# pnnl/nmrfit

Measured on AMD Instinct MI355X. Metric: objective evals/sec (swarm x grid x peaks), higher is better.
Workload: dtype f64

## Files before the change

### nmrfit_amd/csrc/ctx.hip

```cpp
#include "host_call.h"
#include "nmrfit_amd_diag.h"

#include <algorithm>
#include <cmath>
#include <cstdlib>
#include <new>

namespace nmrfit {

int ensure(nmrfit_ctx *ctx, double **buf, int64_t *cap, int64_t need)
{
    if (need <= *cap) return NMRFIT_OK;
    NMRFIT_HIP(hipStreamSynchronize(ctx->stream));
    if (*buf) NMRFIT_HIP(hipFree(*buf));
    *buf = nullptr;
    *cap = 0;
    int64_t n = need + need / 4 + 64;
    NMRFIT_HIP(hipMalloc((void **)buf, (size_t)n * sizeof(double)));
    *cap = n;
    return NMRFIT_OK;
}

void analyse_grid(const double *w, int64_t N, double *w0_out, double *wspan_out, double *lane_step_out, double *grid_dev_out)
{
    const double w0 = w[N / 2];
    double wspan = 0.0, lane_step = 0.0, grid_dev = 0.0;
    for (int64_t j = 0; j < N; ++j) wspan = std::fmax(wspan, std::fabs(w[j] - w0));
    if (N >= 2 * kChunk) {
        const double first = w[0] - w0, step = ((w[N - 1] - w0) - first) / (double)(N - 1);
        double dev = 0.0;
        for (int64_t j = 0; j < N; ++j) dev = std::fmax(dev, std::fabs((w[j] - w0) - (first + (double)j * step)));
        if (step != 0.0 && dev <= 1.0e-6 * std::fabs(step)) {
            lane_step = step * kWave;
            grid_dev = 2.0 * dev;
        }
    }
    *w0_out = w0;
    *wspan_out = wspan;
    *lane_step_out = lane_step;
    *grid_dev_out = grid_dev;
}

static bool variant_known(int variant)
{
    return variant == NMRFIT_VARIANT_DEFAULT || variant == NMRFIT_VARIANT_BASELINE || variant == NMRFIT_VARIANT_NOSKIP ||
           variant == NMRFIT_VARIANT_FARFIELD || variant == NMRFIT_VARIANT_NOREC || variant == NMRFIT_VARIANT_FARFIELD32;
}
static bool variant_built(int variant)
{
#ifdef NMRFIT_AB_BUILD
    return variant_known(variant);
#else
    return variant == NMRFIT_VARIANT_DEFAULT || variant == NMRFIT_VARIANT_FARFIELD || variant == NMRFIT_VARIANT_NOREC ||
           variant == NMRFIT_VARIANT_FARFIELD32;
#endif
}

}

using namespace nmrfit;

#pragma GCC visibility push(default)
extern "C" {

int nmrfit_ctx_create(int device, int64_t N, const double *w, const double *u, const double *v,
                      const double *weights, nmrfit_ctx **out)
{
    if (!out) {
        set_error("null out pointer");
        return NMRFIT_E_INVALID;
    }
    *out = nullptr;
    if (N <= 0 || !w || !u || !v || !weights) {
        set_error("nmrfit_ctx_create: N must be > 0 and w, u, v, weights non-null");
        return NMRFIT_E_INVALID;
    }
    DeviceInfo prop;
    int rc = use_device(device, &prop);
    if (rc != NMRFIT_OK) return rc;
    nmrfit_ctx *ctx = new (std::nothrow) nmrfit_ctx();
    if (!ctx) {
        set_error("out of host memory");
        return NMRFIT_E_INVALID;
    }
    ctx->device = device;
    ctx->compute_units = prop.cus;
    ctx->N = N;
    ctx->n_chunks = block_plan(N).n_chunks;
    if (const char *tw = getenv("NMRFIT_TARGET_WAVES")) ctx->target_waves = atoll(tw);
    if (getenv("NMRFIT_NO_WIDE_WORKGROUPS")) ctx->wide_workgroups = false;
    if (const char *dv = getenv("NMRFIT_DEFAULT_VARIANT")) {
        const int vnum = atoi(dv);
        if (variant_built(vnum)) ctx->variant = vnum;
    }
    analyse_grid(w, N, &ctx->w0, &ctx->wspan, &ctx->lane_step, &ctx->grid_dev);
    const size_t bytes = (size_t)N * sizeof(double);
    const size_t padded = (size_t)ctx->n_chunks * kChunk * sizeof(double);
    NMRFIT_HIP_OR(take_stream(device, &ctx->own_stream), nmrfit_ctx_destroy(ctx));
    ctx->stream = ctx->own_stream;
    NMRFIT_HIP_OR(hipEventCreate(&ctx->ev0), nmrfit_ctx_destroy(ctx));
    NMRFIT_HIP_OR(hipEventCreate(&ctx->ev1), nmrfit_ctx_destroy(ctx));
    Carver c;
    const size_t o_wc = c.take(padded), o_u = c.take(padded), o_v = c.take(padded), o_wt = c.take(padded);
    const size_t o_chunk = c.take((size_t)ctx->n_chunks * sizeof(double2)), o_stage = c.take(bytes);
    NMRFIT_HIP_OR(hipMalloc((void **)&ctx->d_block, c.total), nmrfit_ctx_destroy(ctx));
    NMRFIT_HIP_OR(hipMemsetAsync(ctx->d_block, 0, o_chunk, ctx->stream), nmrfit_ctx_destroy(ctx));
    unsigned char *base = reinterpret_cast<unsigned char *>(ctx->d_block);
    ctx->d_wc = reinterpret_cast<double *>(base + o_wc);
    ctx->d_u = reinterpret_cast<double *>(base + o_u);
    ctx->d_v = reinterpret_cast<double *>(base + o_v);
    ctx->d_wt = reinterpret_cast<double *>(base + o_wt);
    ctx->d_chunk = reinterpret_cast<double2 *>(base + o_chunk);
    ctx->d_stage = reinterpret_cast<double *>(base + o_stage);
    NMRFIT_HIP_OR(hipMemcpyAsync(ctx->d_stage, w, bytes, hipMemcpyHostToDevice, ctx->stream), nmrfit_ctx_destroy(ctx));
    rc = prepare_grid(ctx, ctx->d_stage);
    const double *host_arrays[] = {u, v, weights};
    double *dev_arrays[] = {ctx->d_u, ctx->d_v, ctx->d_wt};
    for (int a = 0; a < 3 && rc == NMRFIT_OK; ++a) {
        NMRFIT_HIP_OR(hipMemcpyAsync(ctx->d_stage, host_arrays[a], bytes, hipMemcpyHostToDevice, ctx->stream),
                      nmrfit_ctx_destroy(ctx));
        rc = scatter_grid(ctx, ctx->d_stage, dev_arrays[a]);
    }
    if (rc != NMRFIT_OK) {
        nmrfit_ctx_destroy(ctx);
        return rc;
    }
    NMRFIT_HIP_OR(hipStreamSynchronize(ctx->stream), nmrfit_ctx_destroy(ctx));
    *out = ctx;
    return NMRFIT_OK;
}

int nmrfit_ctx_destroy(nmrfit_ctx *ctx)
{
    if (!ctx) return NMRFIT_OK;
    (void)hipSetDevice(ctx->device);
    if (ctx->own_stream) {
        (void)hipStreamSynchronize(ctx->stream);
        if (ctx->stream != ctx->own_stream) (void)hipStreamSynchronize(ctx->own_stream);
    }
    void *bufs[] = {ctx->d_block , ctx->d_X, ctx->d_f, ctx->d_partial, ctx->d_R, ctx->d_lsq};
    for (void *b : bufs)
        if (b) (void)hipFree(b);
    if (ctx->ev0) (void)hipEventDestroy(ctx->ev0);
    if (ctx->ev1) (void)hipEventDestroy(ctx->ev1);
    (void)nmrfit_prof_enable(ctx, 0);
    if (ctx->own_stream) give_stream(ctx->device, ctx->own_stream);
    delete ctx;
    return NMRFIT_OK;
}

int nmrfit_ctx_set_weights(nmrfit_ctx *ctx, const double *weights)
{
    int rc = bind(ctx);
    if (rc != NMRFIT_OK) return rc;
    if (!weights) {
        set_error("null weights");
        return NMRFIT_E_INVALID;
    }
    NMRFIT_HIP(hipMemcpyAsync(ctx->d_stage, weights, (size_t)ctx->N * sizeof(double), hipMemcpyHostToDevice, ctx->stream));
    rc = scatter_grid(ctx, ctx->d_stage, ctx->d_wt);
    if (rc != NMRFIT_OK) return rc;
    NMRFIT_HIP(hipStreamSynchronize(ctx->stream));
    return NMRFIT_OK;
}

int nmrfit_ctx_synchronize(nmrfit_ctx *ctx)
{
    int rc = bind(ctx);
    if (rc != NMRFIT_OK) return rc;
    NMRFIT_HIP(hipStreamSynchronize(ctx->stream));
    return NMRFIT_OK;
}

int nmrfit_ctx_set_stream(nmrfit_ctx *ctx, void *hip_stream)
{
    int rc = bind(ctx);
    if (rc != NMRFIT_OK) return rc;
    NMRFIT_HIP(hipStreamSynchronize(ctx->stream));
    ctx->stream = hip_stream ? (hipStream_t)hip_stream : ctx->own_stream;
    return NMRFIT_OK;
}

int nmrfit_ctx_set_variant(nmrfit_ctx *ctx, int variant)
{
    if (!ctx || !variant_known(variant)) {
        set_error("bad context or variant");
        return NMRFIT_E_INVALID;
    }
    if (!variant_built(variant))
        return refuse(NMRFIT_E_UNSUPPORTED,
                      "this kernel variant is an A/B form: it exists in libnmrfit_amd_ab.so (nmrfit_amd/csrc/build.sh --ab) only");
    ctx->variant = variant;
    return NMRFIT_OK;
}

int nmrfit_ctx_n(const nmrfit_ctx *ctx, int64_t *N)
{
    if (!ctx || !N) {
        set_error("null argument");
        return NMRFIT_E_INVALID;
    }
    *N = ctx->N;
    return NMRFIT_OK;
}

int nmrfit_ctx_set_fit_im(nmrfit_ctx *ctx, int fit_im)
{
    const int rc = check_fit_im(ctx ? fit_im : -1);
    if (rc != NMRFIT_OK) return rc;
    ctx->fit_im = fit_im;
    return NMRFIT_OK;
}

int nmrfit_dev_alloc(nmrfit_ctx *ctx, int64_t bytes, void **dptr)
{
    int rc = bind(ctx);
    if (rc != NMRFIT_OK) return rc;
    if (!dptr || bytes < 0) {
        set_error("bad arguments to nmrfit_dev_alloc");
        return NMRFIT_E_INVALID;
    }
    *dptr = nullptr;
    if (bytes == 0) return NMRFIT_OK;
    NMRFIT_HIP(hipMalloc(dptr, (size_t)bytes));
    return NMRFIT_OK;
}

int nmrfit_dev_free(nmrfit_ctx *ctx, void *dptr)
{
    int rc = bind(ctx);
    if (rc != NMRFIT_OK) return rc;
    if (!dptr) return NMRFIT_OK;
    NMRFIT_HIP(hipStreamSynchronize(ctx->stream));
    NMRFIT_HIP(hipFree(dptr));
    return NMRFIT_OK;
}

static int ctx_memcpy(nmrfit_ctx *ctx, const char *who, void *dst, const void *src, int64_t bytes, hipMemcpyKind kind)
{
    int rc = bind(ctx);
    if (rc != NMRFIT_OK) return rc;
    if (bytes < 0 || (bytes > 0 && (!dst || !src))) return refuse(NMRFIT_E_INVALID, std::string("bad arguments to ") + who);
    if (bytes == 0) return NMRFIT_OK;
// ... 169 lines not shown
```

### nmrfit_amd/csrc/nmrfit_internal.h

```cpp
#pragma once
#include <hip/hip_runtime.h>
#include <stdint.h>
#include <string>
#include <vector>

#include "nmrfit_amd.h"

namespace nmrfit {

constexpr int kWave = 64;
constexpr int kWavesPerBlock = 4;
constexpr int kBlock = kWave * kWavesPerBlock;
#ifndef NMRFIT_POINTS
#define NMRFIT_POINTS 8
#endif
constexpr int kPointsPerLane = NMRFIT_POINTS;
constexpr int kChunk = kWave * kPointsPerLane;
constexpr int kMaxBlocks = 16;
struct BlockPlan {
    int64_t n_chunks;
    int blk_chunks;
    int64_t n_blocks;
    int64_t blk_len;
};
inline BlockPlan block_plan(int64_t N)
{
    BlockPlan p;
    p.n_chunks = (N + kChunk - 1) / kChunk;
    p.blk_chunks = (int)((p.n_chunks + kMaxBlocks - 1) / kMaxBlocks);
    p.n_blocks = (p.n_chunks + p.blk_chunks - 1) / p.blk_chunks;
    p.blk_len = (int64_t)p.blk_chunks * kChunk;
    return p;
}
constexpr int kMaxPeaks = 960;

__host__ __device__ inline int64_t grid_slot(int64_t j)
{
    const int64_t o = j & (int64_t)(kChunk - 1);
    const int64_t l = o & (int64_t)(kWave - 1), q = o >> 6;
    return (j - o) + (q >> 1) * (2 * kWave) + 2 * l + (q & 1);
}
static_assert(kWave == 64 && kPointsPerLane % 2 == 0, "grid_slot assumes wave64 and an even number of points per lane");

__device__ inline void chunk_minmax_wave(const double *wc, int64_t N, int64_t c, int lane, double2 *out)
{
    double lo = INFINITY, hi = -INFINITY;
    for (int q = 0; q < kPointsPerLane; ++q) {
        const int64_t j = c * kChunk + q * kWave + lane;
        if (j < N) {
            const double x = wc[grid_slot(j)];
            lo = fmin(lo, x);
            hi = fmax(hi, x);
        }
    }
    for (int off = 32; off > 0; off >>= 1) {
        lo = fmin(lo, __shfl_down(lo, off, kWave));
        hi = fmax(hi, __shfl_down(hi, off, kWave));
    }
    if (lane == 0) out[c] = make_double2(lo, hi);
}

struct PeakLor {
    double ihw;
    double c;
    double al;
    double ag2;
};
struct PeakFast {
    double ihs;
    double cs;
    double ia;
    double pad;
};
struct PeakWin {
    float lo;
    float hi;
};

void set_error(const std::string &msg);
void analyse_grid(const double *w, int64_t N, double *w0, double *wspan, double *lane_step, double *grid_dev);
struct DeviceInfo {
    bool known = false;
    int cus = 0;
    char arch[64] = {0};
};
int device_info_cached(int device, DeviceInfo *out);
int use_device(int device, DeviceInfo *info = nullptr);
int check_spectra_count(const char *who, int32_t S);
hipError_t take_stream(int device, hipStream_t *out);
void give_stream(int device, hipStream_t s);
int hip_fail(hipError_t e, const char *what, const char *file, int line);
int staged_d2h(int device, hipStream_t st, void *dst_host, const void *src_dev, size_t bytes);

#define NMRFIT_HIP(call)                                                        \
    do {                                                                        \
        hipError_t _e = (call);                                                 \
        if (_e != hipSuccess) return ::nmrfit::hip_fail(_e, #call, __FILE__, __LINE__); \
    } while (0)

struct LaunchGeom {
    int64_t waves = 0;
    int32_t nseg = 1;
    int64_t seg_len = 0;
    int32_t waves_per_workgroup = 4;
};

}

struct nmrfit_ctx {
    int device = -1;
    int compute_units = 0;
    hipStream_t stream = nullptr;
    hipStream_t own_stream = nullptr;
    int64_t N = 0;
    double w0 = 0.0;
    double wspan = 0.0;
    double lane_step = 0.0;
    double grid_dev = 0.0;
    int64_t target_waves = 0;
    bool wide_workgroups = true;
    void *d_block = nullptr;
    double *d_wc = nullptr;
    double *d_u = nullptr, *d_v = nullptr, *d_wt = nullptr;
    double2 *d_chunk = nullptr;
    double *d_stage = nullptr;
    int64_t n_chunks = 0;
    double *d_X = nullptr;
    int64_t cap_X = 0;
    double *d_f = nullptr;
    int64_t cap_f = 0;
    double *d_partial = nullptr;
    int64_t cap_partial = 0;
    double *d_R = nullptr;
    int64_t cap_R = 0;
    double *d_lsq = nullptr;
    int64_t cap_lsq = 0;
    hipEvent_t ev0 = nullptr, ev1 = nullptr;
    int variant = NMRFIT_VARIANT_DEFAULT;
    int fit_im = 0;
    nmrfit::LaunchGeom last;
    int64_t prof_cap = 0;
    std::vector<hipEvent_t> prof_k0, prof_k1, prof_marks;
    int64_t prof_nk = 0, prof_nm = 0;
    unsigned long long *d_clk = nullptr;
};

namespace nmrfit {
struct ObjectiveDeferred {
    bool needed = false;
    const double *partial = nullptr;
    int64_t n_blocks = 0;
    int fit_im = 0;
    bool pbest_done = false;
    bool tail_done = false;
    bool need_flush = false;
};
struct PsoFused;
constexpr int64_t kFusedMaxD = 400;
int launch_objective(nmrfit_ctx *ctx, int64_t S, int32_t P, const double *dX, double *df, double *dR,
                     ObjectiveDeferred *defer = nullptr, const PsoFused *fused = nullptr, int rows_fit_im = 0);
int ensure(nmrfit_ctx *ctx, double **buf, int64_t *cap, int64_t need);
int prepare_grid(nmrfit_ctx *ctx, const double *d_w_raw);
int scatter_grid(nmrfit_ctx *ctx, const double *d_src, double *d_dst);
int comm_all_gather(nmrfit_comm *c, hipStream_t stream, const double *d_send, int64_t n, const double **d_all);
nmrfit_ctx *comm_ctx(const nmrfit_comm *c);
bool comm_attach(nmrfit_comm *c);
void comm_detach(nmrfit_comm *c);
}
```

### nmrfit_amd/csrc/objective.hip

```cpp
#include "objective_launch.h"
#include "objective_lds.h"
#include "objective_math.h"

#include <algorithm>
#include <cmath>
#include <cstdio>
#include <cstdlib>

namespace nmrfit {
namespace {

__global__ void finalize_kernel(const double *__restrict__ partial, int64_t S, int64_t n_chunks, int64_t N,
                                int fit_im, double *__restrict__ f)
{
    const int64_t i = (int64_t)blockIdx.x * blockDim.x + threadIdx.x;
    if (i >= S) return;
    f[i] = finalize_value(partial + i * n_chunks * (fit_im ? 2 : 1), n_chunks, N, fit_im);
}

__global__ void finalize_rows_im_kernel(const double *__restrict__ partial, int64_t S, int64_t n_blocks, int64_t N,
                                        double *__restrict__ f2)
{
    const int64_t i = (int64_t)blockIdx.x * blockDim.x + threadIdx.x;
    if (i >= S) return;
// ... 45 lines not shown
{
    const int64_t N = ctx->N;
    hipLaunchKernelGGL(scatter_grid_kernel, dim3((unsigned)((N + 255) / 256)), dim3(256), 0, ctx->stream, d_src, N, d_dst);
    NMRFIT_HIP(hipGetLastError());
    return NMRFIT_OK;
}

constexpr size_t kStaticLds = kObjectiveStaticLds;
static_assert(kObjectiveStaticLds == (size_t)kWsumsCount * sizeof(double) + 64, "objective_launch.h and objective_math.h disagree");
namespace {
struct ResolvedLds {
    int variant;
    size_t lds;
    unsigned aux_off;
};
constexpr ResolvedLds resolve_lds(int variant, int32_t P, bool residual, int fit_im, int wpb, int slices, int rows)
{
    const bool want32 = variant == NMRFIT_VARIANT_FARFIELD32;
    if (want32) variant = NMRFIT_VARIANT_FARFIELD;
    const int np = P > 1 ? P : 1;
    const size_t room = 160 * 1024 - kStaticLds -
                        (rows ? (size_t)rows * (size_t)(4 + 3 * (int64_t)P) * sizeof(double) + 16 : 0);
    if (variant == NMRFIT_VARIANT_FARFIELD && objective_lds_layout(variant, residual, fit_im, np, wpb, slices).end + 16 > room)
        variant = NMRFIT_VARIANT_DEFAULT;
    if (variant == NMRFIT_VARIANT_DEFAULT && objective_lds_layout(variant, residual, fit_im, np, wpb, slices).end + 16 > room)
        variant = NMRFIT_VARIANT_NOREC;
    const ObjectiveLds at = objective_lds_layout(variant, residual, fit_im, np, wpb, slices);
    if (want32 && variant == NMRFIT_VARIANT_FARFIELD && !residual && fit_im == 0) variant = NMRFIT_VARIANT_FARFIELD32;
    return ResolvedLds{variant, at.end, fit_im != 0 ? (unsigned)at.tab : 0u};
}
struct LdsPin {
    int variant, P;
    size_t lds[24];
};
constexpr LdsPin kLdsPins[] = {
    {NMRFIT_VARIANT_DEFAULT, 1, {2224, 6576, 3248, 12048, 7968, 12320, 8992, 17792, 43808, 48160, 80672, 89472, 2208, 6512, 3232, 11920, 7952, 12256, 8976, 17664, 43792, 48096, 80656, 89344}},
    {NMRFIT_VARIANT_DEFAULT, 6, {2656, 8336, 3680, 15568, 8400, 14080, 9424, 21312, 44240, 49920, 81104, 92992, 2560, 7952, 3584, 14800, 8304, 13696, 9328, 20544, 44144, 49536, 81008, 92224}},
    {NMRFIT_VARIANT_DEFAULT, 32, {4944, 17488, 5968, 33872, 10688, 23232, 11712, 39616, 46528, 59072, 83392, 111296, 4432, 15440, 5456, 29776, 10176, 21184, 11200, 35520, 46016, 57024, 82880, 107200}},
    {NMRFIT_VARIANT_DEFAULT, 33, {5040, 17840, 6064, 34576, 10784, 23584, 11808, 40320, 46624, 59424, 83488, 112000, 4512, 15728, 5536, 30352, 10256, 21472, 11280, 36096, 46096, 57312, 82960, 107776}},
    {NMRFIT_VARIANT_DEFAULT, 132, {13744, 52688, 14768, 104272, 19488, 58432, 20512, 110016, 55328, 94272, 92192, 131008, 11632, 44240, 12656, 87376, 17376, 49984, 18400, 93120, 53216, 85824, 90080, 131008}},
    {NMRFIT_VARIANT_DEFAULT, 133, {13840, 53040, 14864, 104976, 19584, 58784, 20608, 110720, 55424, 94624, 92288, 131328, 11712, 44528, 12736, 87952, 17456, 50272, 18480, 93696, 53296, 86112, 90160, 131328}},
    {NMRFIT_VARIANT_DEFAULT, 452, {41904, 78544, 42928, 155984, 47648, 84288, 48672, 161728, 83488, 120128, 120352, 233408, 34672, 136400, 35696, 155984, 40416, 142144, 41440, 161728, 76256, 120128, 113120, 233408}},
    {NMRFIT_VARIANT_DEFAULT, 606, {55456, 103184, 56480, 205264, 61200, 108928, 62224, 211008, 97040, 144768, 133904, 282688, 45760, 103184, 46784, 205264, 51504, 108928, 52528, 211008, 87344, 144768, 124208, 282688}},
    {NMRFIT_VARIANT_DEFAULT, 960, {86608, 159824, 87632, 318544, 92352, 165568, 93376, 324288, 128192, 201408, 118976, 395968, 71248, 159824, 72272, 318544, 76992, 165568, 78016, 324288, 112832, 201408, 149696, 395968}},
    {NMRFIT_VARIANT_FARFIELD, 1, {37008, 41264, 72848, 81424, 42752, 47008, 78592, 87168, 43776, 48032, 80640, 89216, 36992, 41200, 72832, 81296, 42736, 46944, 78576, 87040, 43760, 47968, 80624, 89088}},
    {NMRFIT_VARIANT_FARFIELD, 6, {37280, 42384, 73120, 83664, 43024, 48128, 78864, 89408, 44048, 49152, 80912, 91456, 37184, 42000, 73024, 82896, 42928, 47744, 78768, 88640, 43952, 48768, 80816, 90688}},
    {NMRFIT_VARIANT_FARFIELD, 32, {38736, 48208, 74576, 95312, 44480, 53952, 80320, 101056, 45504, 54976, 82368, 103104, 38224, 46160, 74064, 91216, 43968, 51904, 79808, 96960, 44992, 52928, 81856, 99008}},
    {NMRFIT_VARIANT_FARFIELD, 33, {38800, 48432, 74640, 95760, 44544, 54176, 80384, 101504, 45568, 55200, 82432, 103552, 38272, 46320, 74112, 91536, 44016, 52064, 79856, 97280, 45040, 53088, 81904, 99328}},
    {NMRFIT_VARIANT_FARFIELD, 132, {44336, 70608, 80176, 140112, 50080, 76352, 85920, 145856, 51104, 77376, 87968, 147904, 42224, 62160, 78064, 123216, 47968, 67904, 83808, 128960, 48992, 68928, 85856, 131008}},
    {NMRFIT_VARIANT_FARFIELD, 133, {44400, 70832, 80240, 140560, 50144, 76576, 85984, 146304, 51168, 77600, 88032, 148352, 42272, 62320, 78112, 123536, 48016, 68064, 83856, 129280, 49040, 69088, 85904, 131328}},
    {NMRFIT_VARIANT_FARFIELD, 452, {62256, 142288, 98096, 155984, 68000, 148032, 103840, 161728, 69024, 149056, 105888, 233408, 55024, 113360, 90864, 155984, 60768, 119104, 96608, 161728, 61792, 120128, 98656, 233408}},
    {NMRFIT_VARIANT_FARFIELD, 606, {70880, 103184, 106720, 205264, 76624, 108928, 112464, 211008, 77648, 144768, 114512, 282688, 61184, 138000, 97024, 205264, 66928, 143744, 102768, 211008, 67952, 144768, 104816, 282688}},
    {NMRFIT_VARIANT_FARFIELD, 960, {90704, 159824, 126544, 318544, 96448, 165568, 132288, 324288, 97472, 201408, 134336, 395968, 75344, 159824, 111184, 318544, 81088, 165568, 116928, 324288, 82112, 201408, 118976, 395968}},
    {NMRFIT_VARIANT_NOREC, 1, {2176, 6384, 3200, 11664, 7920, 12128, 8944, 17408, 43760, 47968, 80624, 89088, 2176, 6384, 3200, 11664, 7920, 12128, 8944, 17408, 43760, 47968, 80624, 89088}},
    {NMRFIT_VARIANT_NOREC, 6, {2368, 7184, 3392, 13264, 8112, 12928, 9136, 19008, 43952, 48768, 80816, 90688, 2368, 7184, 3392, 13264, 8112, 12928, 9136, 19008, 43952, 48768, 80816, 90688}},
    {NMRFIT_VARIANT_NOREC, 32, {3408, 11344, 4432, 21584, 9152, 17088, 10176, 27328, 44992, 52928, 81856, 99008, 3408, 11344, 4432, 21584, 9152, 17088, 10176, 27328, 44992, 52928, 81856, 99008}},
    {NMRFIT_VARIANT_NOREC, 33, {3456, 11504, 4480, 21904, 9200, 17248, 10224, 27648, 45040, 53088, 81904, 99328, 3456, 11504, 4480, 21904, 9200, 17248, 10224, 27648, 45040, 53088, 81904, 99328}},
    {NMRFIT_VARIANT_NOREC, 132, {7408, 27344, 8432, 53584, 13152, 33088, 14176, 59328, 48992, 68928, 85856, 131008, 7408, 27344, 8432, 53584, 13152, 33088, 14176, 59328, 48992, 68928, 85856, 131008}},
    {NMRFIT_VARIANT_NOREC, 133, {7456, 27504, 8480, 53904, 13200, 33248, 14224, 59648, 49040, 69088, 85904, 131328, 7456, 27504, 8480, 53904, 13200, 33248, 14224, 59648, 49040, 69088, 85904, 131328}},
    {NMRFIT_VARIANT_NOREC, 452, {20208, 78544, 21232, 155984, 25952, 84288, 26976, 161728, 61792, 120128, 98656, 233408, 20208, 78544, 21232, 155984, 25952, 84288, 26976, 161728, 61792, 120128, 98656, 233408}},
    {NMRFIT_VARIANT_NOREC, 606, {26368, 103184, 27392, 205264, 32112, 108928, 33136, 211008, 67952, 144768, 104816, 282688, 26368, 103184, 27392, 205264, 32112, 108928, 33136, 211008, 67952, 144768, 104816, 282688}},
    {NMRFIT_VARIANT_NOREC, 960, {40528, 159824, 41552, 318544, 46272, 165568, 47296, 324288, 82112, 201408, 118976, 395968, 40528, 159824, 41552, 318544, 46272, 165568, 47296, 324288, 82112, 201408, 118976, 395968}},
};
constexpr bool lds_pins_hold()
{
    for (const LdsPin &p : kLdsPins) {
        int c = 0;
        for (int residual = 0; residual < 2; ++residual)
            for (int fit_im = 0; fit_im < 3; ++fit_im)
                for (int wpb = kWavesPerBlock; wpb <= kWideWaves; wpb += kWavesPerBlock)
                    for (int slices = 1; slices <= wpb; slices += wpb - 1)
                        if (resolve_lds(p.variant, p.P, residual != 0, fit_im, wpb, slices, 0).lds != p.lds[c++]) return false;
    }
    return true;
}
static_assert(lds_pins_hold(), "objective_lds() moved: the layout of objective_lds.h no longer adds up to the pinned totals");
}
size_t objective_lds(int variant, int32_t P, bool residual, int fit_im, int *variant_out, unsigned *aux_off, int wpb,
                     int slices, int rows)
{
    const ResolvedLds r = resolve_lds(variant, P, residual, fit_im, wpb, slices, rows);
    *variant_out = r.variant;
    *aux_off = r.aux_off;
    return r.lds;
}

int launch_objective(nmrfit_ctx *ctx, int64_t S, int32_t P, const double *dX, double *df, double *dR,
                     ObjectiveDeferred *defer, const PsoFused *fused, int rows_fit_im)
{
    if (defer) *defer = ObjectiveDeferred{};
    const bool rows_im = dR && rows_fit_im != 0;
    if (rows_im && (defer || fused || (rows_fit_im != 1 && rows_fit_im != 2))) {
        set_error("launch_objective: residual rows of both channels take fit_im 1 or 2 and no swarm update");
        return NMRFIT_E_INVALID;
    }
    const int fit_im = rows_im ? rows_fit_im : dR ? 0 : ctx->fit_im;
    if (S == 0) return NMRFIT_OK;
    const int64_t N = ctx->N;
    int64_t target_waves = (int64_t)ctx->compute_units * 4 * 16;
    if (ctx->target_waves > 0) target_waves = ctx->target_waves;
    const BlockPlan bp = block_plan(N);
    const int64_t n_chunks = bp.n_chunks, n_blocks = bp.n_blocks, blk_len = bp.blk_len;
    const int blk_chunks = bp.blk_chunks;
    int64_t nseg = std::max<int64_t>(1, std::min<int64_t>(n_blocks, (target_waves + S - 1) / S));
    static const bool seg_rule_r4 = [] {
        const char *e = getenv("NMRFIT_SEG_RULE");
        return !(e && atoi(e) == 3);
    }();
    if (ctx->target_waves == 0 && seg_rule_r4) {
        const int64_t slots = (int64_t)ctx->compute_units * 4 * 4;
        nseg = std::max<int64_t>(1, std::min<int64_t>(n_blocks, (slots + S - 1) / S));
        if (n_chunks / 4 >= 16) nseg = std::max<int64_t>(nseg, std::min<int64_t>(4, n_blocks));
    }
    if (ctx->target_waves == 0) {
        const int64_t simds = (int64_t)ctx->compute_units * 4;
        while (nseg > 1 && n_chunks / nseg < 2 && S * ((nseg + 1) / 2) >= 2 * simds) nseg = (nseg + 1) / 2;
        if (nseg > 1 && S * nseg > 3 * simds && S * (nseg / 2) < 2 * simds && n_chunks / nseg <= 2) nseg /= 2;
    }
    int64_t seg_len = ((n_blocks + nseg - 1) / nseg) * blk_len;
    nseg = (N + seg_len - 1) / seg_len;
    const int64_t waves = S * nseg;
    int variant = NMRFIT_VARIANT_DEFAULT;
    unsigned aux_off = 0;
    const bool fused_rows = fused && fused->x_in;
    auto tail_fits = [&](unsigned tail, int w) {
        return tail != 0u && S <= (int64_t)kDeferredPerLane * kWave * w;
    };
    auto copies = [&](int w, int *slices, int *rows) {
        const bool one_particle = (nseg % w == 0);
        *slices = one_particle ? 1 : w;
        *rows = !fused_rows ? 0 : !one_particle ? w : (nseg == w && tail_fits(fused->tail, w)) ? 3 : 1;
    };
    int wpb = kWavesPerBlock, slices = 0, rows = 0;
    copies(wpb, &slices, &rows);
    size_t lds = objective_lds(ctx->variant, P, dR != nullptr, fit_im, &variant, &aux_off, wpb, slices, rows);
    if (rows_im && (variant != NMRFIT_VARIANT_DEFAULT || ctx->variant != NMRFIT_VARIANT_DEFAULT)) {
        set_error("residual rows with the imaginary channel exist for the DEFAULT kernel variant only (and while its LDS records fit)");
        return NMRFIT_E_UNSUPPORTED;
    }
    const size_t xrow_bytes = fused_rows ? (size_t)(4 + 3 * (int64_t)P) * sizeof(double) : 0;
    if (nseg == kWideWaves && !dR && fit_im == 0 && has_eight_wave_form(variant) && ctx->wide_workgroups) {
        int v8 = variant, s8 = 0, r8 = 0;
        unsigned aux8 = 0;
        copies(kWideWaves, &s8, &r8);
        const size_t lds8 = objective_lds(ctx->variant, P, false, fit_im, &v8, &aux8, kWideWaves, s8, r8);
        if (v8 == variant && lds8 + kStaticLds + 16 + (size_t)r8 * xrow_bytes <= 160 * 1024) {
            wpb = kWideWaves;
            slices = s8;
            rows = r8;
            lds = lds8;
            aux_off = aux8;
        }
    }
    const int64_t blocks = (waves + wpb - 1) / wpb;
    if (blocks > 0x7fffffffLL) {
        set_error("swarm too large for one launch");
        return NMRFIT_E_INVALID;
    }
    if (lds + kStaticLds + 16 + (size_t)rows * xrow_bytes > 160 * 1024) {
        set_error("too many peaks for the kernel's LDS records (with the imaginary model / the fused swarm update)");
        return NMRFIT_E_UNSUPPORTED;
    }
    PsoFused upd{};
    if (fused && fused->x_in) {
        if (dR || (4 + 3 * (int64_t)P) > kFusedMaxD) {
            set_error("fused swarm update: objective launches with D <= kFusedMaxD only");
            return NMRFIT_E_INVALID;
        }
        upd = *fused;
        lds = (lds + 15) & ~(size_t)15;
        upd.xrow_off = (unsigned)lds;
        lds += (size_t)rows * (size_t)(4 + 3 * (int64_t)P) * sizeof(double);
    }
    const bool direct_f = (nseg == 1 || nseg == wpb);
    if (nseg != wpb) upd.pbest = 0u;
    if (upd.pbest == 0u || !tail_fits(upd.tail, wpb)) upd.tail = 0u;
    if (fused && fused->tail != 0u && fused->pending != 0u && upd.tail == 0u) {
        if (!defer) {
            set_error("launch_objective: pending fold without a deferred-launch record");
            return NMRFIT_E_STATE;
        }
        defer->need_flush = true;
        return NMRFIT_OK;
    }
    double *out = df;
    if (!direct_f) {
        int rc = ensure(ctx, &ctx->d_partial, &ctx->cap_partial, S * n_blocks * (fit_im ? 2 : 1));
        if (rc != NMRFIT_OK) return rc;
        out = ctx->d_partial;
    }
    ObjectiveLaunch la{};
    la.ctx = ctx;
    la.S = S;
    la.P = P;
    la.dX = dX;
    la.out = out;
    la.dR = dR;
    la.nseg = (int)nseg;
    la.seg_len = seg_len;
    la.blk_chunks = blk_chunks;
    la.seg_blocks = (int)(seg_len / blk_len);
    la.n_blocks = (int)n_blocks;
    la.blocks = blocks;
    la.lds = lds;
    la.fit_im = fit_im;
    la.upd = upd;
    la.aux_off = aux_off;
    la.wpb = wpb;
    int rc;
    if (rows_im) {
        rc = launch_objective_rows_im(la);
        if (rc != NMRFIT_OK) return rc;
        if (!direct_f) {
            hipLaunchKernelGGL(finalize_rows_im_kernel, dim3((unsigned)((S + 255) / 256)), dim3(256), 0, ctx->stream,
                               ctx->d_partial, S, n_blocks, N, df);
            NMRFIT_HIP(hipGetLastError());
        }
        ctx->last.waves = waves;
        ctx->last.waves_per_workgroup = wpb;
        ctx->last.nseg = (int32_t)nseg;
        ctx->last.seg_len = seg_len;
        return NMRFIT_OK;
    }
    switch (variant) {
        case NMRFIT_VARIANT_DEFAULT: rc = launch_objective_default(la); break;
        case NMRFIT_VARIANT_FARFIELD: rc = launch_objective_farfield(la); break;
        case NMRFIT_VARIANT_FARFIELD32: rc = launch_objective_farfield32(la); break;
        case NMRFIT_VARIANT_NOREC: rc = launch_objective_norec(la); break;
        default:
#ifdef NMRFIT_AB_BUILD
            rc = launch_objective_ab(variant, la);
#else
            set_error("this kernel variant exists in A/B builds of the library only (-DNMRFIT_AB_BUILD)");
            rc = NMRFIT_E_UNSUPPORTED;
#endif
            break;
    }
    if (rc != NMRFIT_OK) return rc;
    if (defer) defer->pbest_done = upd.x_in != nullptr && upd.pbest != 0u;
    if (defer) defer->tail_done = defer->pbest_done && upd.tail != 0u;
    if (!direct_f && defer) {
        defer->needed = true;
        defer->partial = ctx->d_partial;
        defer->n_blocks = n_blocks;
        defer->fit_im = fit_im;
    } else if (!direct_f) {
        hipLaunchKernelGGL(finalize_kernel, dim3((unsigned)((S + 255) / 256)), dim3(256), 0, ctx->stream,
                           ctx->d_partial, S, n_blocks, N, fit_im, df);
        NMRFIT_HIP(hipGetLastError());
    }
    ctx->last.waves = waves;
    ctx->last.waves_per_workgroup = wpb;
    ctx->last.nseg = (int32_t)nseg;
    ctx->last.seg_len = seg_len;
    return NMRFIT_OK;
}

}
```

### nmrfit_amd/csrc/objective_launch.h

```cpp
#pragma once
#include "nmrfit_internal.h"
#include "pso_update.h"

namespace nmrfit {

struct ObjectiveLaunch {
    nmrfit_ctx *ctx;
    int64_t S;
    int32_t P;
    const double *dX;
    double *out;
    double *dR;
    int nseg;
    int64_t seg_len;
    int blk_chunks;
    int seg_blocks;
    int n_blocks;
    int64_t blocks;
    size_t lds;
    int fit_im;
    PsoFused upd;
    unsigned aux_off;
    int wpb;
};

constexpr bool is_farfield(int variant) { return variant == NMRFIT_VARIANT_FARFIELD || variant == NMRFIT_VARIANT_FARFIELD32; }
constexpr bool has_eight_wave_form(int variant)
{
    return variant == NMRFIT_VARIANT_DEFAULT || is_farfield(variant) || variant == NMRFIT_VARIANT_NOREC;
}
constexpr int kWideWaves = 8;
constexpr size_t kObjectiveStaticLds = (size_t)(2 * kMaxBlocks + 8) * sizeof(double) + 64;

size_t objective_lds(int variant, int32_t P, bool residual, int fit_im, int *variant_out, unsigned *aux_off, int wpb,
                     int slices, int rows);

int launch_objective_default(const ObjectiveLaunch &a);
int launch_objective_farfield(const ObjectiveLaunch &a);
int launch_objective_norec(const ObjectiveLaunch &a);
int launch_objective_farfield32(const ObjectiveLaunch &a);
int launch_objective_rows_im(const ObjectiveLaunch &a);
#ifdef NMRFIT_AB_BUILD
int launch_objective_ab(int variant, const ObjectiveLaunch &a);
#endif

}
```

### nmrfit_amd/csrc/objective_lds.h

```cpp
#pragma once
#include "objective_launch.h"
#include "objective_math.h"

namespace nmrfit {
namespace {

struct ObjectiveLds {
    static constexpr size_t lor = 0;
    size_t win, seeds, shr, lseed, far, grec, lorf, tab, end;
};

constexpr __host__ __device__ ObjectiveLds objective_lds_layout(int variant, bool residual, int fit_im, int P, int wpb, int slices)
{
    ObjectiveLds L{};
    L.win = (size_t)slices * P * sizeof(PeakLor);
    L.seeds = ((size_t)slices * P * (sizeof(PeakLor) + sizeof(PeakWin)) + 15) & ~(size_t)15;
    L.shr = L.seeds + (size_t)wpb * kMaxBlocks * sizeof(double2);
    L.lseed = L.shr + kSharedPrologueBytes;
    L.far = L.lseed + (slices == 1 ? 0 : (size_t)wpb * 2 * kWave * sizeof(double));
    L.grec = L.far + ((is_farfield(variant) || fit_im == 2) ? (size_t)wpb * far_stride(fit_im) * sizeof(double) : 0);
    const bool rec = !residual && (variant == NMRFIT_VARIANT_DEFAULT || is_farfield(variant));
    L.lorf = L.grec + (rec ? (size_t)slices * P * sizeof(double2) : 0);
    L.tab = (L.lorf + (variant == NMRFIT_VARIANT_DEFAULT ? (size_t)slices * P * sizeof(PeakFast) : 0) + 15) & ~(size_t)15;
    L.end = L.tab + (fit_im != 0 ? (size_t)kDawTabCount * sizeof(double) + 16 : 0);
    return L;
}

}
}
```

Baseline: 5515 billion.

## Add paired-particle objective kernel sharing grid and data loads across two particles

Adds a new objective kernel form where each four-wave workgroup evaluates two swarm particles. The grid points and u/v/weight data are loaded once per chunk and reused for both particles' Lorentzian models, and the first particle's accumulator is parked in LDS to limit register pressure. It is enabled by default for the real-channel default variant when the swarm is large enough and the LDS budget fits, with an env override. In exchange it uses more LDS per workgroup, adds LDS round trips for the parked values, and halves the number of workgroups, which could lower occupancy.

```diff
diff --git a/nmrfit_amd/csrc/ctx.hip b/nmrfit_amd/csrc/ctx.hip
--- a/nmrfit_amd/csrc/ctx.hip
+++ b/nmrfit_amd/csrc/ctx.hip
@@ -89,6 +89,7 @@
     ctx->n_chunks = block_plan(N).n_chunks;
     if (const char *tw = getenv("NMRFIT_TARGET_WAVES")) ctx->target_waves = atoll(tw);
     if (getenv("NMRFIT_NO_WIDE_WORKGROUPS")) ctx->wide_workgroups = false;
+    if (const char *pw = getenv("NMRFIT_PAIR_WAVES")) ctx->pair_waves = atoi(pw) != 0 ? 1 : 0;
     if (const char *dv = getenv("NMRFIT_DEFAULT_VARIANT")) {
         const int vnum = atoi(dv);
         if (variant_built(vnum)) ctx->variant = vnum;
diff --git a/nmrfit_amd/csrc/nmrfit_internal.h b/nmrfit_amd/csrc/nmrfit_internal.h
--- a/nmrfit_amd/csrc/nmrfit_internal.h
+++ b/nmrfit_amd/csrc/nmrfit_internal.h
@@ -119,6 +119,7 @@
     double grid_dev = 0.0;
     int64_t target_waves = 0;
     bool wide_workgroups = true;
+    int pair_waves = -1;
     void *d_block = nullptr;
     double *d_wc = nullptr;
     double *d_u = nullptr, *d_v = nullptr, *d_wt = nullptr;
diff --git a/nmrfit_amd/csrc/objective.hip b/nmrfit_amd/csrc/objective.hip
--- a/nmrfit_amd/csrc/objective.hip
+++ b/nmrfit_amd/csrc/objective.hip
@@ -221,12 +221,24 @@
             aux_off = aux8;
         }
     }
-    const int64_t blocks = (waves + wpb - 1) / wpb;
+    bool pair = false;
+    if (variant == NMRFIT_VARIANT_DEFAULT && !dR && fit_im == 0 && nseg == kWavesPerBlock && wpb == kWavesPerBlock &&
+        ctx->pair_waves != 0 && (ctx->pair_waves > 0 || (S / 2) * kWavesPerBlock >= (int64_t)ctx->compute_units * 4 * 4)) {
+        const size_t lds2 = objective_pair_lds_layout(P > 1 ? P : 1).end;
+        if (lds2 + kPairStaticLds + 16 + (size_t)kPairParticles * rows * xrow_bytes <= 160 * 1024) {
+            pair = true;
+            lds = lds2;
+            rows *= kPairParticles;
+            aux_off = 0;
+        }
+    }
+    const size_t static_lds = pair ? kPairStaticLds : kStaticLds;
+    const int64_t blocks = pair ? (S + 1) / 2 : (waves + wpb - 1) / wpb;
     if (blocks > 0x7fffffffLL) {
         set_error("swarm too large for one launch");
         return NMRFIT_E_INVALID;
     }
-    if (lds + kStaticLds + 16 + (size_t)rows * xrow_bytes > 160 * 1024) {
+    if (lds + static_lds + 16 + (size_t)rows * xrow_bytes > 160 * 1024) {
         set_error("too many peaks for the kernel's LDS records (with the imaginary model / the fused swarm update)");
         return NMRFIT_E_UNSUPPORTED;
     }
@@ -276,6 +288,7 @@
     la.upd = upd;
     la.aux_off = aux_off;
     la.wpb = wpb;
+    la.pair = pair;
     int rc;
     if (rows_im) {
         rc = launch_objective_rows_im(la);
@@ -292,7 +305,7 @@
         return NMRFIT_OK;
     }
     switch (variant) {
-        case NMRFIT_VARIANT_DEFAULT: rc = launch_objective_default(la); break;
+        case NMRFIT_VARIANT_DEFAULT: rc = pair ? launch_objective_pair(la) : launch_objective_default(la); break;
         case NMRFIT_VARIANT_FARFIELD: rc = launch_objective_farfield(la); break;
         case NMRFIT_VARIANT_FARFIELD32: rc = launch_objective_farfield32(la); break;
         case NMRFIT_VARIANT_NOREC: rc = launch_objective_norec(la); break;
@@ -318,7 +331,7 @@
                            ctx->d_partial, S, n_blocks, N, fit_im, df);
         NMRFIT_HIP(hipGetLastError());
     }
-    ctx->last.waves = waves;
+    ctx->last.waves = pair ? blocks * wpb : waves;
     ctx->last.waves_per_workgroup = wpb;
     ctx->last.nseg = (int32_t)nseg;
     ctx->last.seg_len = seg_len;
diff --git a/nmrfit_amd/csrc/objective_launch.h b/nmrfit_amd/csrc/objective_launch.h
--- a/nmrfit_amd/csrc/objective_launch.h
+++ b/nmrfit_amd/csrc/objective_launch.h
@@ -22,6 +22,7 @@
     PsoFused upd;
     unsigned aux_off;
     int wpb;
+    bool pair;
 };
 
 constexpr bool is_farfield(int variant) { return variant == NMRFIT_VARIANT_FARFIELD || variant == NMRFIT_VARIANT_FARFIELD32; }
@@ -40,6 +41,7 @@
 int launch_objective_norec(const ObjectiveLaunch &a);
 int launch_objective_farfield32(const ObjectiveLaunch &a);
 int launch_objective_rows_im(const ObjectiveLaunch &a);
+int launch_objective_pair(const ObjectiveLaunch &a);
 #ifdef NMRFIT_AB_BUILD
 int launch_objective_ab(int variant, const ObjectiveLaunch &a);
 #endif
diff --git a/nmrfit_amd/csrc/objective_lds.h b/nmrfit_amd/csrc/objective_lds.h
--- a/nmrfit_amd/csrc/objective_lds.h
+++ b/nmrfit_amd/csrc/objective_lds.h
@@ -26,5 +26,32 @@
     return L;
 }
 
+struct ObjectivePairLds {
+    static constexpr size_t lor = 0;
+    size_t lorf, grec, win, seeds, shr, park, state, end;
+};
+constexpr int kPairParticles = 2;
+constexpr size_t kPairParkBytes = (size_t)kPointsPerLane * sizeof(double) * kWave;
+constexpr size_t kPairStateBytes = (size_t)kPairParticles * 3 * sizeof(double) * kWave;
+
+constexpr __host__ __device__ ObjectivePairLds objective_pair_lds_layout(int P)
+{
+    ObjectivePairLds L{};
+    const size_t n = (size_t)kPairParticles * P;
+    L.lorf = n * sizeof(PeakLor);
+    L.grec = L.lorf + n * sizeof(PeakFast);
+    L.win = L.grec + n * sizeof(double2);
+    L.seeds = (L.win + n * sizeof(PeakWin) + 15) & ~(size_t)15;
+    L.shr = L.seeds + (size_t)kPairParticles * kWavesPerBlock * kMaxBlocks * sizeof(double2);
+    L.park = L.shr + (size_t)kPairParticles * kSharedPrologueBytes;
+    L.state = L.park + (size_t)kWavesPerBlock * kPairParkBytes;
+    L.end = L.state + (size_t)kWavesPerBlock * kPairStateBytes;
+    return L;
+}
+constexpr size_t kPairStaticLds = (size_t)kPairParticles * kWsumsCount * sizeof(double) + 64;
+static_assert(kSharedPrologueBytes % 16 == 0 && sizeof(PeakLor) % 16 == 0 && sizeof(PeakFast) % 16 == 0, "16-byte pieces");
+static_assert(objective_pair_lds_layout(24).end + 16 + (size_t)kPairParticles * (4 + 3 * 24) * sizeof(double) + kPairStaticLds <= 40 * 1024,
+              "pair form: four workgroups no longer fit on a CU at P = 24");
+
 }
 }
diff --git a/nmrfit_amd/csrc/objective_pair.h b/nmrfit_amd/csrc/objective_pair.h
--- /dev/null
+++ b/nmrfit_amd/csrc/objective_pair.h
@@ -0,0 +1,372 @@
+#pragma once
+#include "objective_chunk.h"
+#include "objective_finish.h"
+#include "objective_launch.h"
+#include "objective_lds.h"
+#include "objective_prologue.h"
+#include "swarm_prologue.h"
+
+#include <type_traits>
+
+namespace nmrfit {
+namespace {
+
+struct PairSide {
+    PeakLor *lor;
+    PeakFast *lorf;
+    double2 *grec;
+    PeakWin *win;
+    double2 *seeds;
+    double *shr;
+    double *state;
+    double *wsums;
+    double base;
+    bool rec_all;
+};
+
+template <bool FAST, bool FULL>
+__device__ __forceinline__ void pair_model(const PairSide &s, const int P, const int lane, const double2 mm,
+                                           const double (&wv)[kPointsPerLane], double (&acc)[kPointsPerLane])
+{
+    const double base = s.base;
+    int k = 0;
+    {
+        const int kend0 = (P < kWave) ? P : kWave;
+        if (kGroupSize <= kend0) {
+            if constexpr (FAST)
+                lorentz_group_fast<kGroupSize, true>(s.lorf, wv, acc, base);
+            else
+                lorentz_group<kGroupSize, true>(s.lor, wv, acc, base);
+            k = kGroupSize;
+        } else if (kend0 > 0) {
+            if constexpr (FAST)
+                lorentz_tail_fast<true>(kend0, s.lorf, wv, acc, base);
+            else
+                lorentz_tail<kGroupSize, true>(kend0, s.lor, wv, acc, base);
+            k = kend0;
+        } else {
+#pragma unroll
+            for (int q = 0; q < kPointsPerLane; ++q) acc[q] = base;
+        }
+    }
+    for (int kb = 0; kb < P; kb += kWave) {
+        const int kend = (P < kb + kWave) ? P : kb + kWave;
+        bool h = false;
+        if (kb + lane < P) {
+            const PeakWin wn = s.win[kb + lane];
+            h = (mm.y >= (double)wn.lo) && (mm.x <= (double)wn.hi);
+        }
+        unsigned long long hits = __ballot(h);
+        if (kb != 0) k = kb;
+        if constexpr (FAST) {
+            for (; k + kGroupSize <= kend; k += kGroupSize) lorentz_group_fast<kGroupSize>(s.lorf + k, wv, acc);
+            if (k < kend) lorentz_tail_fast(kend - k, s.lorf + k, wv, acc);
+        } else {
+            for (; k + kGroupSize <= kend; k += kGroupSize) lorentz_group<kGroupSize>(s.lor + k, wv, acc);
+            if (k < kend) lorentz_tail<kGroupSize>(kend - k, s.lor + k, wv, acc);
+        }
+        if (kend - kb < kWave) hits &= (1ull << (kend - kb)) - 1ull;
+        const bool rec = FULL && s.rec_all;
+        for (unsigned long long m = rec ? hits : 0ull; m; m &= m - 1) {
+            const int k1 = kb + __builtin_ctzll(m);
+            gauss_add_rec(s.lor + k1, s.grec + k1, wv, acc);
+        }
+        for (unsigned long long m = rec ? 0ull : hits; m; m &= m - 1) gauss_add<true>(s.lor + kb + __builtin_ctzll(m), wv, acc);
+    }
+}
+
+struct PairState {
+    double zr, zi, bs;
+};
+__device__ __forceinline__ PairState pair_state(const PairSide &s, const int lane, const bool first, const int bidx)
+{
+    PairState st;
+    if (first) {
+        const double2 e = s.seeds[bidx];
+        const double lr = s.shr[2 + lane], li = s.shr[2 + kWave + lane];
+        st.zr = __builtin_fma(e.x, lr, -(e.y * li));
+        st.zi = __builtin_fma(e.x, li, e.y * lr);
+    } else {
+        st.zr = s.state[lane];
+        st.zi = s.state[kWave + lane];
+    }
+    st.bs = s.state[2 * kWave + lane];
+    return st;
+}
+
+__device__ __forceinline__ void pair_epilogue(const PairSide &s, const int lane, const PairState &st, const bool last, const int slot,
+                                              const double (&acc)[kPointsPerLane], const double (&uq)[kPointsPerLane],
+                                              const double (&vq)[kPointsPerLane], const double (&tq)[kPointsPerLane])
+{
+    double zr = st.zr, zi = st.zi, bs = st.bs;
+    const double rr = s.shr[0], ri = s.shr[1];
+#pragma unroll
+    for (int q = 0; q < kPointsPerLane; ++q) {
+        const double vd = __builtin_fma(zr, uq[q], -(zi * vq[q]));
+        const double e = tq[q] * (vd - acc[q]);
+        bs = __builtin_fma(e, e, bs);
+        const double nzr = __builtin_fma(zr, rr, -(zi * ri));
+        zi = __builtin_fma(zr, ri, zi * rr);
+        zr = nzr;
+    }
+    if (last) {
+        const double cs = wave_sum(bs);
+        bs = 0.0;
+        if (lane == 0) s.wsums[slot] = cs;
+    }
+    s.state[lane] = zr;
+    s.state[kWave + lane] = zi;
+    s.state[2 * kWave + lane] = bs;
+}
+
+template <int WPB>
+__device__ __forceinline__ void objective_pair_body(
+    unsigned char *lds_raw, double *wsums2, const double *__restrict__ wc, const double *__restrict__ u,
+    const double *__restrict__ v, const double *__restrict__ wt, const double2 *__restrict__ chunk_minmax,
+    const double *__restrict__ X, int64_t S, int P, int64_t N, double w0, double wspan, int64_t seg_len, int blk_chunks,
+    int seg_blocks, int n_blocks_i, double lane_step, double rec_devk, double *__restrict__ out,
+    unsigned long long *__restrict__ clk, const PsoFused &upd)
+{
+    static_assert(WPB == kWavesPerBlock, "the pair layout is sized for four-wave workgroups");
+    const int lane = threadIdx.x & (kWave - 1);
+    const int wave = __builtin_amdgcn_readfirstlane((int)(threadIdx.x >> 6));
+    const ObjectivePairLds at = objective_pair_lds_layout(P);
+    int64_t part[kPairParticles] = {2 * (int64_t)blockIdx.x, 2 * (int64_t)blockIdx.x + 1};
+    const bool hasB = part[1] < S;
+    const int64_t D = 4 + 3 * (int64_t)P;
+    const bool fused = upd.x_in != nullptr;
+    const int rows = (upd.tail != 0u) ? 3 : 1;
+    double *xrow[kPairParticles];
+    PairSide side[kPairParticles];
+    int *sflag[kPairParticles];
+#pragma unroll
+    for (int h = 0; h < kPairParticles; ++h) {
+        side[h].lor = reinterpret_cast<PeakLor *>(lds_raw + ObjectivePairLds::lor) + (size_t)h * P;
+        side[h].lorf = reinterpret_cast<PeakFast *>(lds_raw + at.lorf) + (size_t)h * P;
+        side[h].grec = reinterpret_cast<double2 *>(lds_raw + at.grec) + (size_t)h * P;
+        side[h].win = reinterpret_cast<PeakWin *>(lds_raw + at.win) + (size_t)h * P;
+        side[h].seeds = reinterpret_cast<double2 *>(lds_raw + at.seeds) + ((size_t)h * WPB + wave) * kMaxBlocks;
+        side[h].shr = reinterpret_cast<double *>(lds_raw + at.shr + (size_t)h * kSharedPrologueBytes);
+        side[h].state = reinterpret_cast<double *>(lds_raw + at.state + (size_t)wave * kPairStateBytes) + (size_t)h * 3 * kWave;
+        side[h].wsums = wsums2 + (size_t)h * kWsumsCount;
+        sflag[h] = reinterpret_cast<int *>(side[h].shr + 2 + 2 * kWave);
+        xrow[h] = reinterpret_cast<double *>(lds_raw + upd.xrow_off) + (size_t)h * rows * D;
+    }
+    f64x2 *const park = reinterpret_cast<f64x2 *>(lds_raw + at.park + (size_t)wave * kPairParkBytes);
+    phase_stamp(clk, 0);
+    if (clk && blockIdx.x == 0 && wave == 0 && lane == 0) {
+        clk[0] = __builtin_amdgcn_s_memtime();
+        clk[1] = __builtin_amdgcn_s_memrealtime();
+    }
+    if (fused) {
+        const bool stopped = swarm_prologue<WPB>(upd, xrow[0], D, S, part[0], wave, true, true, wave, lane, side[0].wsums, clk);
+        if (hasB) swarm_prologue<WPB>(upd, xrow[1], D, S, part[1], wave, true, true, wave, lane, side[1].wsums, clk);
+        if (stopped) return;
+    }
+    const double invN = 1.0 / (double)N;
+    double p1[kPairParticles] = {0.0, 0.0};
+#pragma unroll
+    for (int h = 0; h < kPairParticles; ++h) {
+        if (h == 1 && !hasB) break;
+        double p0, r, yoff;
+        bool fast_bad = false, rec_bad = false;
+        const StagePeakConstants<true, true> stage_peaks{p0, p1[h], r, yoff, P, lane, w0, wspan, side[h].lor, side[h].win, fast_bad,
+                                                         side[h].lorf, lane_step, rec_devk, rec_bad, side[h].grec};
+        const int turn = (wave + 2 * h) & (WPB - 1);
+        if (fused)
+            stage_peaks(xrow[h], turn, WPB);
+        else
+            stage_peaks(X + part[h] * D, turn, WPB);
+        if (turn == WPB - 1) {
+            double sr, si, tr, ti;
+            sincos_fast((p1[h] * 64.0) * invN, &si, &sr);
+            sincos_fast(p0 + (p1[h] * (double)lane) * invN, &ti, &tr);
+            if (lane == 0) {
+                side[h].shr[0] = sr;
+                side[h].shr[1] = si;
+            }
+            side[h].shr[2 + lane] = tr;
+            side[h].shr[2 + kWave + lane] = ti;
+        }
+        const int fl = (__ballot(fast_bad) != 0ull ? 1 : 0) | (__ballot(rec_bad) != 0ull ? 2 : 0);
+        if (lane == 0) sflag[h][wave] = fl;
+        side[h].base = wave_uniform((double)P * yoff);
+    }
+    __syncthreads();
+    bool fast_all[kPairParticles] = {true, true};
+#pragma unroll
+    for (int h = 0; h < kPairParticles; ++h) {
+        side[h].rec_all = false;
+        if (h == 1 && !hasB) break;
+        int all = 0;
+#pragma unroll
+        for (int w2 = 0; w2 < WPB; ++w2) all |= sflag[h][w2];
+        fast_all[h] = !(all & 1);
+        side[h].rec_all = !(all & 2);
+    }
+    phase_stamp(clk, 2);
+
+    const int seg = wave;
+    const int64_t j0 = (int64_t)seg * seg_len;
+    const int64_t j1 = (j0 + seg_len < N) ? j0 + seg_len : N;
+    const int64_t blk_len = (int64_t)blk_chunks * kChunk;
+    const int64_t n_blocks = n_blocks_i;
+    const int64_t b0 = (int64_t)seg * seg_blocks;
+    const int64_t nb = (seg_blocks < n_blocks - b0) ? seg_blocks : n_blocks - b0;
+#pragma unroll
+    for (int h = 0; h < kPairParticles; ++h) {
+        if (h == 1 && !hasB) break;
+        if (lane < nb) {
+            double er, ei;
+            sincos_fast((p1[h] * (double)((b0 + lane) * blk_len)) * invN, &ei, &er);
+            side[h].seeds[lane] = make_double2(er, ei);
+        }
+        side[h].state[2 * kWave + lane] = 0.0;
+    }
+    wave_lds_fence();
+    const int blk0 = (int)b0;
+    int cib = 0, bidx = 0;
+
+    auto chunk = [&](const int64_t jb, const bool doA, const bool doB, auto fast_tag, auto full_tag) {
+        constexpr bool kFastLoop = decltype(fast_tag)::value;
+        constexpr bool full = decltype(full_tag)::value;
+        const int64_t jl = jb + lane;
+        double wv[kPointsPerLane], accA[kPointsPerLane], accB[kPointsPerLane];
+        double uq[kPointsPerLane], vq[kPointsPerLane], tq[kPointsPerLane];
+        if (full) {
+            const global_pairs wp = lane_ptr(wc + jb, lane);
+#pragma unroll
+            for (int m = 0; m < kPointsPerLane / 2; ++m) {
+                const f64x2 d = wp[m * kWave];
+                wv[2 * m] = d.x;
+                wv[2 * m + 1] = d.y;
+            }
+        } else {
+#pragma unroll
+            for (int q = 0; q < kPointsPerLane; ++q)
+                wv[q] = (jl + q * kWave < j1) ? wc[jb + (q >> 1) * (2 * kWave) + 2 * lane + (q & 1)] : 0.0;
+        }
+        const double2 mm = global_table(chunk_minmax, jb / kChunk);
+        if (doA) {
+            pair_model<kFastLoop, full>(side[0], P, lane, mm, wv, accA);
+#pragma unroll
+            for (int m = 0; m < kPointsPerLane / 2; ++m) park[m * kWave + lane] = f64x2{accA[2 * m], accA[2 * m + 1]};
+        }
+        if (doB) pair_model<kFastLoop, full>(side[1], P, lane, mm, wv, accB);
+        asm volatile("" ::: "memory");
+        if (full) {
+            const global_pairs up = lane_ptr(u + jb, lane), vp = lane_ptr(v + jb, lane), tp = lane_ptr(wt + jb, lane);
+#pragma unroll
+            for (int m = 0; m < kPointsPerLane / 2; ++m) {
+                const f64x2 du = up[m * kWave], dv = vp[m * kWave], dt = tp[m * kWave];
+                uq[2 * m] = du.x;
+                uq[2 * m + 1] = du.y;
+                vq[2 * m] = dv.x;
+                vq[2 * m + 1] = dv.y;
+                tq[2 * m] = dt.x;
+                tq[2 * m + 1] = dt.y;
+            }
+        } else {
+#pragma unroll
+            for (int q = 0; q < kPointsPerLane; ++q) {
+                const bool ok = jl + q * kWave < j1;
+                const int64_t js = jb + (q >> 1) * (2 * kWave) + 2 * lane + (q & 1);
+                uq[q] = ok ? u[js] : 0.0;
+                vq[q] = ok ? v[js] : 0.0;
+                tq[q] = ok ? wt[js] : 0.0;
+            }
+        }
+        const bool first = cib == 0;
+        const bool last = (cib + 1 == blk_chunks) || (jb + kChunk >= j1);
+        if (doB) pair_epilogue(side[1], lane, pair_state(side[1], lane, first, bidx), last, blk0 + bidx, accB, uq, vq, tq);
+        if (doA) {
+            wave_lds_fence();
+#pragma unroll
+            for (int m = 0; m < kPointsPerLane / 2; ++m) {
+                const f64x2 d = park[m * kWave + lane];
+                accA[2 * m] = d.x;
+                accA[2 * m + 1] = d.y;
+            }
+            pair_epilogue(side[0], lane, pair_state(side[0], lane, first, bidx), last, blk0 + bidx, accA, uq, vq, tq);
+        }
+        wave_lds_fence();
+        ++cib;
+        if (last) {
+            cib = 0;
+            ++bidx;
+        }
+    };
+    auto chunk_loop = [&](const bool doA, const bool doB, auto fast_tag) {
+        cib = 0;
+        bidx = 0;
+        int64_t jb = j0;
+        for (; jb + kChunk <= j1; jb += kChunk) chunk(jb, doA, doB, fast_tag, std::true_type{});
+        if (jb < j1) chunk(jb, doA, doB, fast_tag, std::false_type{});
+    };
+    if (fast_all[0] && fast_all[1]) {
+        chunk_loop(true, hasB, std::true_type{});
+    } else {
+        if (fast_all[0])
+            chunk_loop(true, false, std::true_type{});
+        else
+            chunk_loop(true, false, std::false_type{});
+        if (hasB) {
+            if (fast_all[1])
+                chunk_loop(false, true, std::true_type{});
+            else
+                chunk_loop(false, true, std::false_type{});
+        }
+    }
+
+    phase_stamp(clk, 3);
+    if (clk && blockIdx.x == 0 && wave == 0 && lane == 0) {
+        clk[2] = __builtin_amdgcn_s_memtime();
+        clk[3] = __builtin_amdgcn_s_memrealtime();
+    }
+    __syncthreads();
+#pragma unroll
+    for (int h = 0; h < kPairParticles; ++h) {
+        if (wave != h || (h == 1 && !hasB)) continue;
+        double *wsums = side[h].wsums;
+        if (lane == 0) {
+            double t = 0.0;
+            for (int64_t c = 0; c < n_blocks; ++c) t += wsums[c];
+            const double f = sqrt(t / (double)N);
+            out[part[h]] = f;
+            wsums[2 * kMaxBlocks] = f;
+        }
+        wave_lds_fence();
+        phase_stamp(clk, 4);
+        const PersonalBest<false> personal_best{wsums, P, part[h], lds_raw, clk};
+        personal_best(wsums[2 * kMaxBlocks]);
+    }
+}
+
+template <int WPB = kWavesPerBlock>
+__global__ __launch_bounds__(kWave *WPB, kMinWaves) void objective_kernel_pair(
+    const double *__restrict__ wc, const double *__restrict__ u, const double *__restrict__ v,
+    const double *__restrict__ wt, const double2 *__restrict__ chunk_minmax, const double *__restrict__ X, int64_t S,
+    int P, int64_t N, double w0, double wspan, int64_t seg_len, int blk_chunks, int seg_blocks, int n_blocks,
+    double lane_step, double rec_devk, double *__restrict__ out, unsigned long long *__restrict__ clk, const PsoFused upd)
+{
+    extern __shared__ __align__(16) unsigned char lds_raw[];
+    __shared__ double wsums2[kPairParticles * kWsumsCount];
+    if (threadIdx.x < kPairParticles) {
+        const int h = threadIdx.x;
+        double *wsums = wsums2 + h * kWsumsCount;
+        const int64_t particle = 2 * (int64_t)blockIdx.x + h;
+        const int64_t D = 4 + 3 * (int64_t)P;
+        const bool pbest = upd.x_in != nullptr && upd.pbest != 0u;
+        wsums[2 * kMaxBlocks + 1] = pbest ? 1.0 : 0.0;
+        wsums[2 * kMaxBlocks + 2] = __longlong_as_double((long long)(uintptr_t)upd.p);
+        wsums[2 * kMaxBlocks + 3] = __longlong_as_double((long long)S);
+        wsums[2 * kMaxBlocks + 4] = __longlong_as_double((long long)(upd.xrow_off + (unsigned)h * (upd.tail != 0u ? 3u : 1u) * (unsigned)(D * sizeof(double))));
+        if (pbest && particle < S) wsums[2 * kMaxBlocks + 5] = upd.p[S * D + particle];
+        wsums[2 * kMaxBlocks + 7] = __longlong_as_double((pbest && upd.tail != 0u) ? (long long)upd.pflip : 0LL);
+    }
+    objective_pair_body<WPB>(lds_raw, wsums2, wc, u, v, wt, chunk_minmax, X, S, P, N, w0, wspan, seg_len, blk_chunks, seg_blocks,
+                             n_blocks, lane_step, rec_devk, out, clk, upd);
+}
+
+}
+}
diff --git a/nmrfit_amd/csrc/objective_pair.hip b/nmrfit_amd/csrc/objective_pair.hip
--- /dev/null
+++ b/nmrfit_amd/csrc/objective_pair.hip
@@ -0,0 +1,27 @@
+#include "objective_pair.h"
+
+namespace nmrfit {
+
+int launch_objective_pair(const ObjectiveLaunch &a)
+{
+    nmrfit_ctx *const ctx = a.ctx;
+    if (a.dR || a.fit_im != 0 || a.nseg != kWavesPerBlock || a.wpb != kWavesPerBlock || !a.pair) {
+        set_error("internal: the pair form takes objective launches of the real channel with four segments per particle");
+        return NMRFIT_E_STATE;
+    }
+    const bool prof = ctx->prof_cap > 0 && ctx->prof_nk < ctx->prof_cap;
+    unsigned long long *clk = prof ? ctx->d_clk : nullptr;
+    if (prof) NMRFIT_HIP(hipEventRecord(ctx->prof_k0[(size_t)ctx->prof_nk], ctx->stream));
+    hipLaunchKernelGGL((objective_kernel_pair<kWavesPerBlock>), dim3((unsigned)a.blocks), dim3(kWave * kWavesPerBlock), a.lds,
+                       ctx->stream, ctx->d_wc, ctx->d_u, ctx->d_v, ctx->d_wt, ctx->d_chunk, a.dX, a.S, (int)a.P, ctx->N, ctx->w0,
+                       ctx->wspan, a.seg_len, a.blk_chunks, a.seg_blocks, a.n_blocks, ctx->lane_step, ctx->grid_dev * 11.0e10,
+                       a.out, clk, a.upd);
+    NMRFIT_HIP(hipGetLastError());
+    if (prof) {
+        NMRFIT_HIP(hipEventRecord(ctx->prof_k1[(size_t)ctx->prof_nk], ctx->stream));
+        ++ctx->prof_nk;
+    }
+    return NMRFIT_OK;
+}
+
+}
```

Result: faster. 5579 billion, median of 6 (+1.2%).
